# lastdancewithyou/multimodal_edema_prediction

Measured on AMD Instinct MI355X. Metric: multimodal train samples/sec, higher is better.
Workload: dtype bf16

## Files before the change

multimodal_edema_prediction_amd/csrc/elementwise.hip:

```cpp
#include "common.h"
#include "medp_hip.h"

namespace {

__global__ __launch_bounds__(256) void cast_f32_bf16_kernel(const float* __restrict__ x, int ldx, bf16_t* __restrict__ y, int ldy,
                                                            int rows, int cols) {
    const int c4 = cols >> 2;
    const size_t total = (size_t)rows * c4;
    for (size_t i = (size_t)blockIdx.x * 256 + threadIdx.x; i < total; i += (size_t)gridDim.x * 256) {
        const int r = (int)(i / c4), c = (int)(i % c4) * 4;
        const float4 v = *(const float4*)(x + (size_t)r * ldx + c);
        uint2 o;
        o.x = pack_bf2(v.x, v.y);
        o.y = pack_bf2(v.z, v.w);
        *(uint2*)(y + (size_t)r * ldy + c) = o;
    }
}

template <typename TIN>
__global__ __launch_bounds__(256) void transpose_to_bf16_kernel(const TIN* __restrict__ x, int ldx, bf16_t* __restrict__ y, int ldy,
                                                                int rows, int cols) {
    __shared__ float tile[64][65];
    const int r0 = blockIdx.y * 64, c0 = blockIdx.x * 64;
    const int tx = threadIdx.x & 63, ty = threadIdx.x >> 6;
    for (int i = ty; i < 64; i += 4) {
        const int r = r0 + i, c = c0 + tx;
        float v = 0.f;
        if (r < rows && c < cols) {
            if constexpr (sizeof(TIN) == 2) v = bf2f(((const bf16_t*)x)[(size_t)r * ldx + c]);
            else v = ((const float*)x)[(size_t)r * ldx + c];
        }
        tile[i][tx] = v;
    }
    __syncthreads();
    for (int i = ty; i < 64; i += 4) {
        const int c = c0 + i, r = r0 + tx;
        if (c < cols && r < rows) y[(size_t)c * ldy + r] = f2bf(tile[tx][i]);
    }
}

__global__ __launch_bounds__(256) void weight_operands_multi_kernel(const MedpOperandJob* __restrict__ jobs, const int* __restrict__ blk_job,
                                                                    const int* __restrict__ blk_tile) {
    __shared__ float tile[64][65];
    const MedpOperandJob j = jobs[blk_job[blockIdx.x]];
    const int tiles_c = (j.cols + 63) / 64;
    const int t = blk_tile[blockIdx.x];
    const int r0 = (t / tiles_c) * 64, c0 = (t % tiles_c) * 64;
    const int tx = threadIdx.x & 63, ty = threadIdx.x >> 6;
    const float* x = (const float*)j.src;
    bf16_t* yp = (bf16_t*)j.dst_plain;
    bf16_t* yt = (bf16_t*)j.dst_t;
    for (int i = ty; i < 64; i += 4) {
        const int r = r0 + i, c = c0 + tx;
        float v = 0.f;
        if (r < j.rows && c < j.cols) {
            v = x[(size_t)r * j.ld_src + c];
            if (yp) yp[(size_t)r * j.ld_plain + c] = f2bf(v);
        }
        tile[i][tx] = v;
    }
    if (!yt) return;
    __syncthreads();
    for (int i = ty; i < 64; i += 4) {
        const int c = c0 + i, r = r0 + tx;
        if (c < j.cols && r < j.rows) yt[(size_t)c * j.ld_t + r] = f2bf(tile[tx][i]);
    }
}

__global__ __launch_bounds__(256) void gelu_bwd_kernel(const float* __restrict__ dy, const float* __restrict__ pre, float* __restrict__ dx,
                                                       size_t n) {
    for (size_t i = ((size_t)blockIdx.x * 256 + threadIdx.x) * 4; i < n; i += (size_t)gridDim.x * 1024) {
        const float4 g = *(const float4*)(dy + i), p = *(const float4*)(pre + i);
        *(float4*)(dx + i) = make_float4(g.x * gelu_erf_grad(p.x), g.y * gelu_erf_grad(p.y), g.z * gelu_erf_grad(p.z),
                                         g.w * gelu_erf_grad(p.w));
    }
}

__global__ __launch_bounds__(256) void gelu_bf16_fwd_kernel(const bf16_t* __restrict__ pre, bf16_t* __restrict__ out, size_t n8) {
    for (size_t i = (size_t)blockIdx.x * 256 + threadIdx.x; i < n8; i += (size_t)gridDim.x * 256) {
        const uint4 p = *(const uint4*)(pre + i * 8);
        const uint32_t w[4] = {p.x, p.y, p.z, p.w};
        uint32_t o[4];
#pragma unroll
        for (int k = 0; k < 4; ++k) {
            const f32x2 g = gelu_erf2((f32x2){__uint_as_float(w[k] << 16), __uint_as_float(w[k] & 0xffff0000u)});
            o[k] = pack_bf2(g[0], g[1]);
        }
        *(uint4*)(out + i * 8) = make_uint4(o[0], o[1], o[2], o[3]);
    }
}
__global__ __launch_bounds__(256) void gelu_bf16_bwd_kernel(const bf16_t* __restrict__ dy, const bf16_t* __restrict__ pre,
                                                            bf16_t* __restrict__ dx, size_t n8) {
    for (size_t i = (size_t)blockIdx.x * 256 + threadIdx.x; i < n8; i += (size_t)gridDim.x * 256) {
        const uint4 g = *(const uint4*)(dy + i * 8), p = *(const uint4*)(pre + i * 8);
        const uint32_t gw[4] = {g.x, g.y, g.z, g.w}, pw[4] = {p.x, p.y, p.z, p.w};
        uint32_t o[4];
#pragma unroll
        for (int k = 0; k < 4; ++k) {
            const float a = __uint_as_float(gw[k] << 16) * gelu_erf_grad(__uint_as_float(pw[k] << 16));
            const float b = __uint_as_float(gw[k] & 0xffff0000u) * gelu_erf_grad(__uint_as_float(pw[k] & 0xffff0000u));
            o[k] = pack_bf2(a, b);
        }
        *(uint4*)(dx + i * 8) = make_uint4(o[0], o[1], o[2], o[3]);
    }
}

__global__ __launch_bounds__(256) void im2col_patch_kernel(const float* __restrict__ pix, bf16_t* __restrict__ A, int B, int C, int H,
                                                           int W, int ps, int kpad) {
    const unsigned gh = H / ps, gw = W / ps, K = C * ps * ps, pp = ps * ps, k8 = kpad >> 3;
    const unsigned total = (unsigned)B * gh * gw * k8;
    for (unsigned i = blockIdx.x * 256u + threadIdx.x; i < total; i += gridDim.x * 256u) {
        const unsigned kc = i % k8, row = i / k8;
        const unsigned px = row % gw, r2 = row / gw, py = r2 % gh, b = r2 / gh;
        const float* img = pix + (size_t)b * C * H * W + (size_t)(py * ps) * W + px * ps;
        float v[8];
#pragma unroll
        for (int u = 0; u < 8; ++u) {
            const unsigned kk = kc * 8 + u;
            float x = 0.f;
            if (kk < K) {
                const unsigned c = kk / pp, rem = kk - c * pp, ii = rem / ps, jj = rem - ii * ps;
                x = img[((size_t)c * H + ii) * W + jj];
            }
            v[u] = x;
        }
        uint4 o;
        o.x = pack_bf2(v[0], v[1]);
        o.y = pack_bf2(v[2], v[3]);
        o.z = pack_bf2(v[4], v[5]);
        o.w = pack_bf2(v[6], v[7]);
        *(uint4*)(A + (size_t)row * kpad + kc * 8) = o;
    }
}

__global__ __launch_bounds__(256) void vit_assemble_kernel(const float* __restrict__ patch, const float* __restrict__ cls,
                                                           const float* __restrict__ pos, float* __restrict__ x, int B, int P, int D) {
    const int d4 = D >> 2;
    const size_t total = (size_t)B * (P + 1) * d4;
    for (size_t i = (size_t)blockIdx.x * 256 + threadIdx.x; i < total; i += (size_t)gridDim.x * 256) {
        const int c = (int)(i % d4) * 4;
        const size_t tokrow = i / d4;
        const int t = (int)(tokrow % (P + 1)), b = (int)(tokrow / (P + 1));
        const float4 pe = *(const float4*)(pos + (size_t)t * D + c);
        const float4 v = (t == 0) ? *(const float4*)(cls + c) : *(const float4*)(patch + ((size_t)b * P + t - 1) * D + c);
        *(float4*)(x + tokrow * D + c) = make_float4(v.x + pe.x, v.y + pe.y, v.z + pe.z, v.w + pe.w);
    }
}

__device__ __forceinline__ float cubic1(float x, float A) { return ((A + 2.f) * x - (A + 3.f)) * x * x + 1.f; }
__device__ __forceinline__ float cubic2(float x, float A) { return ((A * x - 5.f * A) * x + 8.f * A) * x - 4.f * A; }
__global__ __launch_bounds__(256) void pos_bicubic_kernel(const float* __restrict__ pos, float* __restrict__ out, int s, int gh, int gw,
                                                          int D) {
    const size_t total = (size_t)(gh * gw + 1) * D;
    const float A = -0.75f;
    for (size_t i = (size_t)blockIdx.x * 256 + threadIdx.x; i < total; i += (size_t)gridDim.x * 256) {
        const int d = (int)(i % D), t = (int)(i / D);
        if (t == 0) { out[i] = pos[d]; continue; }
        const int oy = (t - 1) / gw, ox = (t - 1) % gw;
        const float sy = (float)s / (float)gh, sx = (float)s / (float)gw;
        const float fy = (oy + 0.5f) * sy - 0.5f, fx = (ox + 0.5f) * sx - 0.5f;
        const int iy = (int)floorf(fy), ix = (int)floorf(fx);
        const float ty = fy - iy, tx = fx - ix;
        const float wy[4] = {cubic2(ty + 1.f, A), cubic1(ty, A), cubic1(1.f - ty, A), cubic2(2.f - ty, A)};
        const float wx[4] = {cubic2(tx + 1.f, A), cubic1(tx, A), cubic1(1.f - tx, A), cubic2(2.f - tx, A)};
        float acc = 0.f;
#pragma unroll
        for (int a = 0; a < 4; ++a) {
            const int yy = min(max(iy - 1 + a, 0), s - 1);
            float rowacc = 0.f;
#pragma unroll
            for (int c = 0; c < 4; ++c) {
                const int xx = min(max(ix - 1 + c, 0), s - 1);
                rowacc += wx[c] * pos[(size_t)(1 + yy * s + xx) * D + d];
            }
            acc += wy[a] * rowacc;
        }
        out[i] = acc;
    }
}

__device__ __forceinline__ float bicubic_tap_weight(int src, int dst, int s, int g) {
    const float A = -0.75f;
    const float sc = (float)s / (float)g;
    const float f = (dst + 0.5f) * sc - 0.5f;
    const int i0 = (int)floorf(f);
    const float t = f - i0;
    const float w[4] = {cubic2(t + 1.f, A), cubic1(t, A), cubic1(1.f - t, A), cubic2(2.f - t, A)};
    float acc = 0.f;
#pragma unroll
    for (int a = 0; a < 4; ++a)
        if (min(max(i0 - 1 + a, 0), s - 1) == src) acc += w[a];
    return acc;
}
__global__ __launch_bounds__(256) void pos_bicubic_bwd_kernel(const float* __restrict__ dout, float* __restrict__ dpos, int s, int gh,
                                                              int gw, int D) {
    const int d4n = D >> 2;
    const int total = (s * s + 1) * d4n;
    for (int i = blockIdx.x * 256 + threadIdx.x; i < total; i += gridDim.x * 256) {
        const int d4 = i % d4n, cell = i / d4n;
        if (cell == 0) {
            *(float4*)(dpos + 4 * d4) = *(const float4*)(dout + 4 * d4);
            continue;
        }
        const int sy = (cell - 1) / s, sx = (cell - 1) % s;
        float4 acc = make_float4(0.f, 0.f, 0.f, 0.f);
        for (int oy = 0; oy < gh; ++oy) {
            const float wy = bicubic_tap_weight(sy, oy, s, gh);
            if (wy == 0.f) continue;
            for (int ox = 0; ox < gw; ++ox) {
                const float wx = bicubic_tap_weight(sx, ox, s, gw);
                if (wx == 0.f) continue;
                const float w = wy * wx;
                const float4 g = *(const float4*)(dout + (size_t)(1 + oy * gw + ox) * D + 4 * d4);
                acc.x += w * g.x; acc.y += w * g.y; acc.z += w * g.z; acc.w += w * g.w;
            }
        }
        *(float4*)(dpos + (size_t)cell * D + 4 * d4) = acc;
    }
}

inline int grid_for(size_t work_items) { return (int)min((size_t)4096, max((size_t)1, (work_items + 255) / 256)); }

}

extern "C" int medp_cast_f32_bf16(const float* x, int ldx, void* y, int ldy, int rows, int cols, void* stream) {
    MEDP_CHECK_ARG(x && y && rows > 0 && cols > 0, "cast: bad argument");
    MEDP_CHECK_ARG(cols % 4 == 0 && ldx % 4 == 0 && ldy % 4 == 0, "cast: cols, ldx, ldy must be multiples of 4");
    cast_f32_bf16_kernel<<<grid_for((size_t)rows * cols / 4), 256, 0, (hipStream_t)stream>>>(x, ldx, (bf16_t*)y, ldy, rows, cols);
    MEDP_LAUNCH_CHECK("medp_cast_f32_bf16");
    return 0;
}

extern "C" int medp_transpose_to_bf16(const void* x, int x_is_bf16, int ldx, void* y, int ldy, int rows, int cols, void* stream) {
    MEDP_CHECK_ARG(x && y && rows > 0 && cols > 0 && ldx >= cols && ldy >= rows, "transpose: bad argument");
    dim3 grid((cols + 63) / 64, (rows + 63) / 64);
    if (x_is_bf16)
        transpose_to_bf16_kernel<bf16_t><<<grid, 256, 0, (hipStream_t)stream>>>((const bf16_t*)x, ldx, (bf16_t*)y, ldy, rows, cols);
    else
        transpose_to_bf16_kernel<float><<<grid, 256, 0, (hipStream_t)stream>>>((const float*)x, ldx, (bf16_t*)y, ldy, rows, cols);
    MEDP_LAUNCH_CHECK("medp_transpose_to_bf16");
    return 0;
}

extern "C" int medp_weight_operands_multi(const MedpOperandJob* dev_jobs, const int* dev_block_job, const int* dev_block_tile, int n_blocks,
                                          void* stream) {
    MEDP_CHECK_ARG(dev_jobs && dev_block_job && dev_block_tile && n_blocks > 0, "weight_operands_multi: bad argument");
    weight_operands_multi_kernel<<<n_blocks, 256, 0, (hipStream_t)stream>>>(dev_jobs, dev_block_job, dev_block_tile);
    MEDP_LAUNCH_CHECK("medp_weight_operands_multi");
    return 0;
}

extern "C" int medp_gelu_bwd(const float* dy, const float* pre, float* dx, long long n, void* stream) {
    MEDP_CHECK_ARG(dy && pre && dx && n > 0 && n % 4 == 0, "gelu_bwd: bad argument (n must be a multiple of 4)");
    gelu_bwd_kernel<<<grid_for((size_t)n / 4), 256, 0, (hipStream_t)stream>>>(dy, pre, dx, (size_t)n);
    MEDP_LAUNCH_CHECK("medp_gelu_bwd");
    return 0;
}

extern "C" int medp_gelu_bf16_fwd(const void* pre, void* out, long long n, void* stream) {
    MEDP_CHECK_ARG(pre && out && n > 0 && n % 8 == 0, "gelu_bf16_fwd: bad argument (n must be a multiple of 8)");
    gelu_bf16_fwd_kernel<<<grid_for((size_t)n / 8), 256, 0, (hipStream_t)stream>>>((const bf16_t*)pre, (bf16_t*)out, (size_t)n / 8);
    MEDP_LAUNCH_CHECK("medp_gelu_bf16_fwd");
    return 0;
}

extern "C" int medp_gelu_bf16_bwd(const void* dy, const void* pre, void* dx, long long n, void* stream) {
    MEDP_CHECK_ARG(dy && pre && dx && n > 0 && n % 8 == 0, "gelu_bf16_bwd: bad argument (n must be a multiple of 8)");
    gelu_bf16_bwd_kernel<<<grid_for((size_t)n / 8), 256, 0, (hipStream_t)stream>>>((const bf16_t*)dy, (const bf16_t*)pre, (bf16_t*)dx,
                                                                                  (size_t)n / 8);
    MEDP_LAUNCH_CHECK("medp_gelu_bf16_bwd");
    return 0;
}

extern "C" int medp_im2col_patch(const float* pix, void* A, int B, int C, int H, int W, int patch, int kpad, void* stream) {
    MEDP_CHECK_ARG(pix && A && B > 0 && C > 0 && patch > 0, "im2col: bad argument");
    MEDP_CHECK_ARG(H >= patch && W >= patch, "im2col: image %dx%d smaller than the patch size %d", H, W, patch);
    MEDP_CHECK_ARG(kpad >= C * patch * patch && kpad % 8 == 0, "im2col: kpad must be >= C*p*p and a multiple of 8");
    const size_t total = (size_t)B * (H / patch) * (W / patch) * (kpad / 8);
    MEDP_CHECK_ARG(total < (1ull << 31), "im2col: B * patches * kpad / 8 must stay below 2^31");
    im2col_patch_kernel<<<grid_for(total), 256, 0, (hipStream_t)stream>>>(pix, (bf16_t*)A, B, C, H, W, patch, kpad);
    MEDP_LAUNCH_CHECK("medp_im2col_patch");
    return 0;
}

extern "C" int medp_vit_assemble(const float* patch, const float* cls, const float* pos, float* x, int B, int P, int D, void* stream) {
    MEDP_CHECK_ARG(patch && cls && pos && x && B > 0 && P > 0 && D % 4 == 0, "vit_assemble: bad argument");
    vit_assemble_kernel<<<grid_for((size_t)B * (P + 1) * D / 4), 256, 0, (hipStream_t)stream>>>(patch, cls, pos, x, B, P, D);
    MEDP_LAUNCH_CHECK("medp_vit_assemble");
    return 0;
}

extern "C" int medp_pos_embed_bicubic_bwd(const float* dout, float* dpos, int src_side, int gh, int gw, int D, void* stream) {
    MEDP_CHECK_ARG(dout && dpos && src_side > 0 && gh > 0 && gw > 0 && D > 0 && D % 4 == 0, "pos_embed_bicubic_bwd: bad argument");
    pos_bicubic_bwd_kernel<<<grid_for((size_t)(src_side * src_side + 1) * (D / 4)), 256, 0, (hipStream_t)stream>>>(dout, dpos, src_side, gh, gw, D);
    MEDP_LAUNCH_CHECK("medp_pos_embed_bicubic_bwd");
    return 0;
}

extern "C" int medp_pos_embed_bicubic(const float* pos, float* out, int src_side, int gh, int gw, int D, void* stream) {
    MEDP_CHECK_ARG(pos && out && src_side > 0 && gh > 0 && gw > 0 && D > 0, "pos_embed_bicubic: bad argument");
    pos_bicubic_kernel<<<grid_for((size_t)(gh * gw + 1) * D), 256, 0, (hipStream_t)stream>>>(pos, out, src_side, gh, gw, D);
    MEDP_LAUNCH_CHECK("medp_pos_embed_bicubic");
    return 0;
}
```

multimodal_edema_prediction_amd/csrc/norm.hip:

```cpp
#include <stdlib.h>

#include "common.h"
#include "medp_hip.h"

namespace {

template <bool OUT_BF16>
__global__ __launch_bounds__(256) void layernorm_fwd_kernel(const float* __restrict__ x, int ldx, const float* __restrict__ w,
                                                            const float* __restrict__ b, void* __restrict__ y, int ldy,
                                                            float* __restrict__ mean_out, float* __restrict__ rstd_out,
                                                            int rows, int D, float eps) {
    const int lane = threadIdx.x & 63;
    const int row = blockIdx.x * 4 + (threadIdx.x >> 6);
    if (row >= rows) return;
    const float* xr = x + (size_t)row * ldx;
    const int D4 = D >> 2;
    float s = 0.f;
    for (int i = lane; i < D4; i += 64) {
        const float4 v = *(const float4*)(xr + 4 * i);
        s += (v.x + v.y) + (v.z + v.w);
    }
    const float mean = wave_sum(s) / (float)D;
    float ss = 0.f;
    for (int i = lane; i < D4; i += 64) {
        const float4 v = *(const float4*)(xr + 4 * i);
        const float a = v.x - mean, c = v.y - mean, d = v.z - mean, e = v.w - mean;
        ss += (a * a + c * c) + (d * d + e * e);
    }
    const float rstd = rsqrtf(wave_sum(ss) / (float)D + eps);
    if (lane == 0) {
        if (mean_out) mean_out[row] = mean;
        if (rstd_out) rstd_out[row] = rstd;
    }
    for (int i = lane; i < D4; i += 64) {
        const float4 v = *(const float4*)(xr + 4 * i);
        const float4 ww = *(const float4*)(w + 4 * i);
        const float4 bb = *(const float4*)(b + 4 * i);
        const float o0 = (v.x - mean) * rstd * ww.x + bb.x, o1 = (v.y - mean) * rstd * ww.y + bb.y;
        const float o2 = (v.z - mean) * rstd * ww.z + bb.z, o3 = (v.w - mean) * rstd * ww.w + bb.w;
        if (OUT_BF16) {
            uint2 o;
            o.x = pack_bf2(o0, o1);
            o.y = pack_bf2(o2, o3);
            *(uint2*)((bf16_t*)y + (size_t)row * ldy + 4 * i) = o;
        } else {
            *(float4*)((float*)y + (size_t)row * ldy + 4 * i) = make_float4(o0, o1, o2, o3);
        }
    }
}

template <bool OUT_BF16, int NV>
__global__ __launch_bounds__(256) void layernorm_fwd_reg_kernel(const float* __restrict__ x, int ldx, const float* __restrict__ w,
                                                                const float* __restrict__ b, void* __restrict__ y, int ldy,
                                                                float* __restrict__ mean_out, float* __restrict__ rstd_out,
                                                                int rows, float eps) {
    constexpr int D = 256 * NV;
    const int lane = threadIdx.x & 63;
    const int row = blockIdx.x * 4 + (threadIdx.x >> 6);
    if (row >= rows) return;
    const float* xr = x + (size_t)row * ldx;
    float4 v[NV];
#pragma unroll
    for (int j = 0; j < NV; ++j) v[j] = *(const float4*)(xr + 4 * (lane + 64 * j));
    float s = 0.f;
#pragma unroll
    for (int j = 0; j < NV; ++j) s += (v[j].x + v[j].y) + (v[j].z + v[j].w);
    const float mean = wave_sum(s) / (float)D;
    float ss = 0.f;
#pragma unroll
    for (int j = 0; j < NV; ++j) {
        const float a = v[j].x - mean, c = v[j].y - mean, d = v[j].z - mean, e = v[j].w - mean;
        ss += (a * a + c * c) + (d * d + e * e);
    }
    const float rstd = rsqrtf(wave_sum(ss) / (float)D + eps);
    if (lane == 0) {
        if (mean_out) mean_out[row] = mean;
        if (rstd_out) rstd_out[row] = rstd;
    }
#pragma unroll
    for (int j = 0; j < NV; ++j) {
        const int i = lane + 64 * j;
        const float4 ww = *(const float4*)(w + 4 * i);
        const float4 bb = *(const float4*)(b + 4 * i);
        const float o0 = (v[j].x - mean) * rstd * ww.x + bb.x, o1 = (v[j].y - mean) * rstd * ww.y + bb.y;
        const float o2 = (v[j].z - mean) * rstd * ww.z + bb.z, o3 = (v[j].w - mean) * rstd * ww.w + bb.w;
        if (OUT_BF16) {
            uint2 o;
            o.x = pack_bf2(o0, o1);
            o.y = pack_bf2(o2, o3);
            *(uint2*)((bf16_t*)y + (size_t)row * ldy + 4 * i) = o;
        } else {
            *(float4*)((float*)y + (size_t)row * ldy + 4 * i) = make_float4(o0, o1, o2, o3);
        }
    }
}

__global__ __launch_bounds__(256) void layernorm_bwd_dx_kernel(const float* __restrict__ dy, int lddy, const float* __restrict__ x,
                                                               int ldx, const float* __restrict__ w, const float* __restrict__ mean,
                                                               const float* __restrict__ rstd, float* __restrict__ dx, int lddx,
                                                               int rows, int D, int accumulate) {
    const int lane = threadIdx.x & 63;
    const int row = blockIdx.x * 4 + (threadIdx.x >> 6);
    if (row >= rows) return;
    const float* xr = x + (size_t)row * ldx;
    const float* gr = dy + (size_t)row * lddy;
    const float mu = mean[row], rs = rstd[row];
    const int D4 = D >> 2;
    float s1 = 0.f, s2 = 0.f;
    for (int i = lane; i < D4; i += 64) {
        const float4 v = *(const float4*)(xr + 4 * i), g = *(const float4*)(gr + 4 * i), ww = *(const float4*)(w + 4 * i);
        const float g0 = g.x * ww.x, g1 = g.y * ww.y, g2 = g.z * ww.z, g3 = g.w * ww.w;
        s1 += (g0 + g1) + (g2 + g3);
        s2 += (g0 * (v.x - mu) + g1 * (v.y - mu)) + (g2 * (v.z - mu) + g3 * (v.w - mu));
    }
    s1 = wave_sum(s1) / (float)D;
    s2 = wave_sum(s2) * rs / (float)D;
    float* dr = dx + (size_t)row * lddx;
    for (int i = lane; i < D4; i += 64) {
        const float4 v = *(const float4*)(xr + 4 * i), g = *(const float4*)(gr + 4 * i), ww = *(const float4*)(w + 4 * i);
        float4 o;
        o.x = rs * (g.x * ww.x - s1 - (v.x - mu) * rs * s2);
        o.y = rs * (g.y * ww.y - s1 - (v.y - mu) * rs * s2);
        o.z = rs * (g.z * ww.z - s1 - (v.z - mu) * rs * s2);
        o.w = rs * (g.w * ww.w - s1 - (v.w - mu) * rs * s2);
        if (accumulate) {
            const float4 old = *(const float4*)(dr + 4 * i);
            o.x += old.x; o.y += old.y; o.z += old.z; o.w += old.w;
        }
        *(float4*)(dr + 4 * i) = o;
    }
}

template <int MODE>
__global__ __launch_bounds__(256) void colsum_partial_kernel(const float* __restrict__ dy, int lddy, const float* __restrict__ x, int ldx,
                                                             const float* __restrict__ mean, const float* __restrict__ rstd,
                                                             float* __restrict__ partial, int rows, int D, int rows_per_chunk) {
    __shared__ float red[2][4][64];
    const int cl = threadIdx.x & 63, rl = threadIdx.x >> 6;
    const int c = blockIdx.x * 64 + cl;
    const int chunk = blockIdx.y, nchunk = gridDim.y;
    const int r0 = chunk * rows_per_chunk, r1 = min(rows, r0 + rows_per_chunk);
    float a = 0.f, bsum = 0.f;
    if (c < D) {
        for (int r = r0 + rl; r < r1; r += 4) {
            const float g = dy[(size_t)r * lddy + c];
            bsum += g;
            if (MODE == 1) a += g * (x[(size_t)r * ldx + c] - mean[r]) * rstd[r];
        }
    }
    red[0][rl][cl] = a;
    red[1][rl][cl] = bsum;
    __syncthreads();
    if (rl == 0 && c < D) {
        if (MODE == 1) partial[(size_t)chunk * D + c] = (red[0][0][cl] + red[0][1][cl]) + (red[0][2][cl] + red[0][3][cl]);
        partial[(size_t)(nchunk + chunk) * D + c] = (red[1][0][cl] + red[1][1][cl]) + (red[1][2][cl] + red[1][3][cl]);
    }
}

__global__ __launch_bounds__(256) void colsum_final_kernel(const float* __restrict__ partial, float* __restrict__ out_a,
                                                           float* __restrict__ out_b, int nchunk, int D) {
    __shared__ float red[2][4][64];
    const int cl = threadIdx.x & 63, kl = threadIdx.x >> 6;
    const int c = blockIdx.x * 64 + cl;
    float a = 0.f, b = 0.f;
    if (c < D) {
#pragma unroll 4
        for (int k = kl; k < nchunk; k += 4) {
            if (out_a) a += partial[(size_t)k * D + c];
            b += partial[(size_t)(nchunk + k) * D + c];
        }
    }
    red[0][kl][cl] = a;
    red[1][kl][cl] = b;
    __syncthreads();
    if (kl == 0 && c < D) {
        if (out_a) out_a[c] = (red[0][0][cl] + red[0][1][cl]) + (red[0][2][cl] + red[0][3][cl]);
        if (out_b) out_b[c] = (red[1][0][cl] + red[1][1][cl]) + (red[1][2][cl] + red[1][3][cl]);
    }
}

template <bool OUT_BF16>
__global__ __launch_bounds__(256) void scalenorm_fwd_kernel(const float* __restrict__ x, int ldx, const float* __restrict__ g,
                                                            void* __restrict__ y, int ldy, float* __restrict__ rnorm_out, int rows,
                                                            int D, float eps) {
    const int lane = threadIdx.x & 63;
    const int row = blockIdx.x * 4 + (threadIdx.x >> 6);
    if (row >= rows) return;
    const float* xr = x + (size_t)row * ldx;
    const int D4 = D >> 2;
    float ss = 0.f;
    for (int i = lane; i < D4; i += 64) {
        const float4 v = *(const float4*)(xr + 4 * i);
        ss += (v.x * v.x + v.y * v.y) + (v.z * v.z + v.w * v.w);
    }
    const float rn = 1.0f / fmaxf(sqrtf(wave_sum(ss)), eps);
    if (lane == 0 && rnorm_out) rnorm_out[row] = rn;
    const float sc = rn * sqrtf((float)D) * g[0];
    for (int i = lane; i < D4; i += 64) {
        const float4 v = *(const float4*)(xr + 4 * i);
        if (OUT_BF16) {
            uint2 o;
            o.x = pack_bf2(v.x * sc, v.y * sc);
            o.y = pack_bf2(v.z * sc, v.w * sc);
            *(uint2*)((bf16_t*)y + (size_t)row * ldy + 4 * i) = o;
        } else {
            *(float4*)((float*)y + (size_t)row * ldy + 4 * i) = make_float4(v.x * sc, v.y * sc, v.z * sc, v.w * sc);
        }
    }
}

template <bool OUT_BF16, int NV>
__global__ __launch_bounds__(256) void scalenorm_fwd_reg_kernel(const float* __restrict__ x, int ldx, const float* __restrict__ g,
                                                                void* __restrict__ y, int ldy, float* __restrict__ rnorm_out,
                                                                int rows, int D, float eps) {
    const int lane = threadIdx.x & 63;
    const int row = blockIdx.x * 4 + (threadIdx.x >> 6);
    if (row >= rows) return;
    const float* xr = x + (size_t)row * ldx;
    const int D4 = D >> 2;
    float4 v[NV];
#pragma unroll
    for (int k = 0; k < NV; ++k) {
        const int i = lane + 64 * k;
        v[k] = i < D4 ? *(const float4*)(xr + 4 * i) : make_float4(0.f, 0.f, 0.f, 0.f);
    }
    float ss = 0.f;
#pragma unroll
    for (int k = 0; k < NV; ++k)
        if (lane + 64 * k < D4) ss += (v[k].x * v[k].x + v[k].y * v[k].y) + (v[k].z * v[k].z + v[k].w * v[k].w);
    const float rn = 1.0f / fmaxf(sqrtf(wave_sum(ss)), eps);
    if (lane == 0 && rnorm_out) rnorm_out[row] = rn;
    const float sc = rn * sqrtf((float)D) * g[0];
#pragma unroll
    for (int k = 0; k < NV; ++k) {
        const int i = lane + 64 * k;
        if (i < D4) {
            if (OUT_BF16) {
                uint2 o;
                o.x = pack_bf2(v[k].x * sc, v[k].y * sc);
                o.y = pack_bf2(v[k].z * sc, v[k].w * sc);
                *(uint2*)((bf16_t*)y + (size_t)row * ldy + 4 * i) = o;
            } else {
                *(float4*)((float*)y + (size_t)row * ldy + 4 * i) = make_float4(v[k].x * sc, v[k].y * sc, v[k].z * sc, v[k].w * sc);
            }
        }
    }
}

__global__ __launch_bounds__(256) void scalenorm_bwd_kernel(const float* __restrict__ dy, int lddy, const float* __restrict__ x, int ldx,
                                                            const float* __restrict__ g, const float* __restrict__ rnorm, const float* acc_src,
                                                            int ldacc, float* dx, int lddx, float* dg_rows, int rows, int D) {
    const int lane = threadIdx.x & 63;
    const int row = blockIdx.x * 4 + (threadIdx.x >> 6);
    if (row >= rows) return;
    {
        const float* xr = x + (size_t)row * ldx;
        const float* gr = dy + (size_t)row * lddy;
        const int D4 = D >> 2;
        float dot = 0.f;
        for (int i = lane; i < D4; i += 64) {
            const float4 v = *(const float4*)(xr + 4 * i), d = *(const float4*)(gr + 4 * i);
            dot += (v.x * d.x + v.y * d.y) + (v.z * d.z + v.w * d.w);
        }
        dot = wave_sum(dot);
        const float rn = rnorm[row], sq = sqrtf((float)D);
        if (lane == 0 && dg_rows) dg_rows[row] = sq * rn * dot;
        const float s = sq * g[0] * rn, k = rn * rn * dot;
        float* dr = dx + (size_t)row * lddx;
        for (int i = lane; i < D4; i += 64) {
            const float4 v = *(const float4*)(xr + 4 * i), d = *(const float4*)(gr + 4 * i);
            float4 o = make_float4(s * (d.x - v.x * k), s * (d.y - v.y * k), s * (d.z - v.z * k), s * (d.w - v.w * k));
            if (acc_src) {
                const float4 old = *(const float4*)(acc_src + (size_t)row * ldacc + 4 * i);
                o.x += old.x; o.y += old.y; o.z += old.z; o.w += old.w;
            }
            *(float4*)(dr + 4 * i) = o;
        }
    }
}

template <int NV>
__global__ __launch_bounds__(256) void scalenorm_bwd_reg_kernel(const float* __restrict__ dy, int lddy, const float* __restrict__ x, int ldx,
                                                                const float* __restrict__ g, const float* __restrict__ rnorm,
                                                                const float* acc_src, int ldacc, float* dx, int lddx, float* dg_rows, int rows,
                                                                int D) {
    const int lane = threadIdx.x & 63;
    const int row = blockIdx.x * 4 + (threadIdx.x >> 6);
    if (row >= rows) return;
    {
        const float* xr = x + (size_t)row * ldx;
        const float* gr = dy + (size_t)row * lddy;
        const int D4 = D >> 2;
        float4 v[NV], d[NV];
        float dot = 0.f;
#pragma unroll
        for (int j = 0; j < NV; ++j) {
            const int i = lane + 64 * j;
            const bool ok = i < D4;
            v[j] = ok ? *(const float4*)(xr + 4 * i) : make_float4(0.f, 0.f, 0.f, 0.f);
            d[j] = ok ? *(const float4*)(gr + 4 * i) : make_float4(0.f, 0.f, 0.f, 0.f);
        }
#pragma unroll
        for (int j = 0; j < NV; ++j) dot += (v[j].x * d[j].x + v[j].y * d[j].y) + (v[j].z * d[j].z + v[j].w * d[j].w);
        dot = wave_sum(dot);
        const float rn = rnorm[row], sq = sqrtf((float)D);
        if (lane == 0 && dg_rows) dg_rows[row] = sq * rn * dot;
        const float s = sq * g[0] * rn, k = rn * rn * dot;
        float* dr = dx + (size_t)row * lddx;
#pragma unroll
        for (int j = 0; j < NV; ++j) {
            const int i = lane + 64 * j;
            if (i < D4) {
                float4 o = make_float4(s * (d[j].x - v[j].x * k), s * (d[j].y - v[j].y * k), s * (d[j].z - v[j].z * k), s * (d[j].w - v[j].w * k));
                if (acc_src) {
                    const float4 old = *(const float4*)(acc_src + (size_t)row * ldacc + 4 * i);
                    o.x += old.x; o.y += old.y; o.z += old.z; o.w += old.w;
                }
                *(float4*)(dr + 4 * i) = o;
            }
        }
    }
}

__global__ __launch_bounds__(256) void sum_all_kernel(const float* __restrict__ v, float* __restrict__ out, int n) {
    __shared__ float red[4];
    float s = 0.f;
    for (int i = threadIdx.x; i < n; i += 256) s += v[i];
    s = wave_sum(s);
    if ((threadIdx.x & 63) == 0) red[threadIdx.x >> 6] = s;
    __syncthreads();
    if (threadIdx.x == 0) out[0] = (red[0] + red[1]) + (red[2] + red[3]);
}

int colsum_chunks(int rows) { return max(1, min(128, rows / 64)); }

constexpr int COLSUM_DIRECT_MAX_ROWS = 2048;
template <int MODE>
__global__ __launch_bounds__(1024) void colsum_direct_kernel(const float* __restrict__ dy, int lddy, const float* __restrict__ x, int ldx,
                                                            const float* __restrict__ mean, const float* __restrict__ rstd,
                                                            float* __restrict__ out_a, float* __restrict__ out_b, int rows, int D) {
    __shared__ float red[2][16][64];
    const int cl = threadIdx.x & 63, rl = threadIdx.x >> 6;
    const int c = blockIdx.x * 64 + cl;
    float a = 0.f, bsum = 0.f;
    if (c < D) {
#pragma unroll 4
        for (int r = rl; r < rows; r += 16) {
            const float g = dy[(size_t)r * lddy + c];
            bsum += g;
            if (MODE == 1) a += g * (x[(size_t)r * ldx + c] - mean[r]) * rstd[r];
        }
    }
    red[0][rl][cl] = a;
    red[1][rl][cl] = bsum;
    __syncthreads();
    if (rl == 0 && c < D) {
        float sa = 0.f, sb = 0.f;
#pragma unroll
        for (int k = 0; k < 16; ++k) {
            sa += red[0][k][cl];
            sb += red[1][k][cl];
        }
        if (MODE == 1 && out_a) out_a[c] = sa;
        if (out_b) out_b[c] = sb;
    }
}

}

extern "C" int medp_layernorm_fwd(const float* x, int ldx, const float* w, const float* b, void* y, int ldy, int y_bf16,
                                  float* mean, float* rstd, int rows, int D, float eps, void* stream) {
    MEDP_CHECK_ARG(x && w && b && y, "layernorm_fwd: null operand");
    MEDP_CHECK_ARG(rows > 0 && D > 0 && D % 4 == 0 && ldx % 4 == 0 && ldy % 4 == 0, "layernorm_fwd: D, ldx, ldy must be multiples of 4");
    dim3 grid((rows + 3) / 4);
    hipStream_t s = (hipStream_t)stream;
    if (D == 768 && y_bf16)
        layernorm_fwd_reg_kernel<true, 3><<<grid, 256, 0, s>>>(x, ldx, w, b, y, ldy, mean, rstd, rows, eps);
    else if (D == 768)
        layernorm_fwd_reg_kernel<false, 3><<<grid, 256, 0, s>>>(x, ldx, w, b, y, ldy, mean, rstd, rows, eps);
    else if (D == 256 && y_bf16)
        layernorm_fwd_reg_kernel<true, 1><<<grid, 256, 0, s>>>(x, ldx, w, b, y, ldy, mean, rstd, rows, eps);
    else if (D == 256)
        layernorm_fwd_reg_kernel<false, 1><<<grid, 256, 0, s>>>(x, ldx, w, b, y, ldy, mean, rstd, rows, eps);
    else if (y_bf16)
        layernorm_fwd_kernel<true><<<grid, 256, 0, s>>>(x, ldx, w, b, y, ldy, mean, rstd, rows, D, eps);
    else
        layernorm_fwd_kernel<false><<<grid, 256, 0, s>>>(x, ldx, w, b, y, ldy, mean, rstd, rows, D, eps);
    MEDP_LAUNCH_CHECK("medp_layernorm_fwd");
    return 0;
}

extern "C" size_t medp_colsum_workspace_bytes(int rows, int D) { return (size_t)2 * colsum_chunks(rows) * D * sizeof(float); }

extern "C" int medp_layernorm_bwd(const float* dy, int lddy, const float* x, int ldx, const float* w, const float* mean,
                                  const float* rstd, float* dx, int lddx, int accumulate_dx, float* dw, float* db,
                                  float* workspace, int rows, int D, void* stream) {
    MEDP_CHECK_ARG(dy && x && w && mean && rstd, "layernorm_bwd: null operand");
    MEDP_CHECK_ARG(rows > 0 && D > 0 && D % 4 == 0 && ldx % 4 == 0 && lddy % 4 == 0 && lddx % 4 == 0, "layernorm_bwd: alignment");
    hipStream_t s = (hipStream_t)stream;
    if (dx) {
        layernorm_bwd_dx_kernel<<<(rows + 3) / 4, 256, 0, s>>>(dy, lddy, x, ldx, w, mean, rstd, dx, lddx, rows, D, accumulate_dx);
        MEDP_LAUNCH_CHECK("medp_layernorm_bwd(dx)");
    }
    if (dw || db) {
        MEDP_CHECK_ARG(workspace, "layernorm_bwd: workspace required for dw/db (medp_colsum_workspace_bytes)");
        if (rows <= COLSUM_DIRECT_MAX_ROWS) {
            colsum_direct_kernel<1><<<(D + 63) / 64, 1024, 0, s>>>(dy, lddy, x, ldx, mean, rstd, dw, db, rows, D);
            MEDP_LAUNCH_CHECK("medp_layernorm_bwd(direct)");
            return 0;
        }
        const int nchunk = colsum_chunks(rows), rpc = (rows + nchunk - 1) / nchunk;
        colsum_partial_kernel<1><<<dim3((D + 63) / 64, nchunk), 256, 0, s>>>(dy, lddy, x, ldx, mean, rstd, workspace, rows, D, rpc);
        MEDP_LAUNCH_CHECK("medp_layernorm_bwd(partial)");
        colsum_final_kernel<<<(D + 63) / 64, 256, 0, s>>>(workspace, dw, db, nchunk, D);
        MEDP_LAUNCH_CHECK("medp_layernorm_bwd(final)");
    }
    return 0;
}

extern "C" int medp_colsum_f32(const float* x, int ldx, float* out, float* workspace, int rows, int D, void* stream) {
    MEDP_CHECK_ARG(x && out && workspace && rows > 0 && D > 0, "colsum: bad argument");
    hipStream_t s = (hipStream_t)stream;
    if (rows <= COLSUM_DIRECT_MAX_ROWS) {
        colsum_direct_kernel<0><<<(D + 63) / 64, 1024, 0, s>>>(x, ldx, nullptr, 0, nullptr, nullptr, nullptr, out, rows, D);
        MEDP_LAUNCH_CHECK("medp_colsum_f32(direct)");
        return 0;
    }
    const int nchunk = colsum_chunks(rows), rpc = (rows + nchunk - 1) / nchunk;
    colsum_partial_kernel<0><<<dim3((D + 63) / 64, nchunk), 256, 0, s>>>(x, ldx, nullptr, 0, nullptr, nullptr, workspace, rows, D, rpc);
    MEDP_LAUNCH_CHECK("medp_colsum_f32(partial)");
    colsum_final_kernel<<<(D + 63) / 64, 256, 0, s>>>(workspace, nullptr, out, nchunk, D);
    MEDP_LAUNCH_CHECK("medp_colsum_f32(final)");
    return 0;
}

extern "C" int medp_scalenorm_fwd(const float* x, int ldx, const float* g, void* y, int ldy, int y_bf16, float* rnorm, int rows,
                                  int D, float eps, void* stream) {
    MEDP_CHECK_ARG(x && g && y, "scalenorm_fwd: null operand");
    MEDP_CHECK_ARG(rows > 0 && D > 0 && D % 4 == 0 && ldx % 4 == 0 && ldy % 4 == 0, "scalenorm_fwd: D, ldx, ldy must be multiples of 4");
    dim3 grid((rows + 3) / 4);
    const int nv = (D / 4 + 63) / 64;
    hipStream_t st = (hipStream_t)stream;
#define MEDP_SN_REG(NV)                                                                                             \
    do {                                                                                                            \
        if (y_bf16) scalenorm_fwd_reg_kernel<true, NV><<<grid, 256, 0, st>>>(x, ldx, g, y, ldy, rnorm, rows, D, eps);  \
        else scalenorm_fwd_reg_kernel<false, NV><<<grid, 256, 0, st>>>(x, ldx, g, y, ldy, rnorm, rows, D, eps);       \
    } while (0)
    if (nv <= 2) MEDP_SN_REG(2);
    else if (nv <= 5) MEDP_SN_REG(5);
    else if (nv <= 10) MEDP_SN_REG(10);
    else if (nv <= 16) MEDP_SN_REG(16);
    else if (y_bf16)
        scalenorm_fwd_kernel<true><<<grid, 256, 0, st>>>(x, ldx, g, y, ldy, rnorm, rows, D, eps);
    else
        scalenorm_fwd_kernel<false><<<grid, 256, 0, st>>>(x, ldx, g, y, ldy, rnorm, rows, D, eps);
#undef MEDP_SN_REG
    MEDP_LAUNCH_CHECK("medp_scalenorm_fwd");
    return 0;
}

static int scalenorm_bwd_launch(const float* dy, int lddy, const float* x, int ldx, const float* g, const float* rnorm, const float* acc_src,
                                int ldacc, float* dx, int lddx, float* dg, float* workspace_rows, int rows, int D, void* stream) {
    MEDP_CHECK_ARG(dy && x && g && rnorm && dx, "scalenorm_bwd: null operand");
    MEDP_CHECK_ARG(rows > 0 && D % 4 == 0 && ldx % 4 == 0 && lddy % 4 == 0 && lddx % 4 == 0 && ldacc % 4 == 0, "scalenorm_bwd: alignment");
    MEDP_CHECK_ARG(!dg || workspace_rows, "scalenorm_bwd: dg needs a rows-float workspace");
    hipStream_t s = (hipStream_t)stream;
    const int nv = (D / 4 + 63) / 64;
    float* dgr = dg ? workspace_rows : nullptr;
    const int grid = (rows + 3) / 4;
    if (nv <= 5) scalenorm_bwd_reg_kernel<5><<<grid, 256, 0, s>>>(dy, lddy, x, ldx, g, rnorm, acc_src, ldacc, dx, lddx, dgr, rows, D);
    else if (nv <= 10) scalenorm_bwd_reg_kernel<10><<<grid, 256, 0, s>>>(dy, lddy, x, ldx, g, rnorm, acc_src, ldacc, dx, lddx, dgr, rows, D);
    else scalenorm_bwd_kernel<<<grid, 256, 0, s>>>(dy, lddy, x, ldx, g, rnorm, acc_src, ldacc, dx, lddx, dgr, rows, D);
    MEDP_LAUNCH_CHECK("medp_scalenorm_bwd");
    if (dg) {
        sum_all_kernel<<<1, 256, 0, s>>>(workspace_rows, dg, rows);
        MEDP_LAUNCH_CHECK("medp_scalenorm_bwd(dg)");
    }
    return 0;
}

extern "C" int medp_scalenorm_bwd(const float* dy, int lddy, const float* x, int ldx, const float* g, const float* rnorm, float* dx,
                                  int lddx, int accumulate_dx, float* dg, float* workspace_rows, int rows, int D, void* stream) {
    return scalenorm_bwd_launch(dy, lddy, x, ldx, g, rnorm, accumulate_dx ? dx : nullptr, lddx, dx, lddx, dg, workspace_rows, rows, D, stream);
}

extern "C" int medp_scalenorm_bwd_add(const float* dy, int lddy, const float* x, int ldx, const float* g, const float* rnorm, const float* add,
                                      int ldadd, float* dx, int lddx, float* dg, float* workspace_rows, int rows, int D, void* stream) {
    MEDP_CHECK_ARG(add, "scalenorm_bwd_add: null operand");
    return scalenorm_bwd_launch(dy, lddy, x, ldx, g, rnorm, add, ldadd, dx, lddx, dg, workspace_rows, rows, D, stream);
}
```

Measured before the change: 12580.

## Add specialized patch-14 im2col and optional pipelined multi-row LayerNorm forward

Adds an im2col kernel specialized for patch size 14 that reads float2 pairs with incremental index stepping instead of per-element div/mod, enabled by default through an env variable. Also adds a persistent, software-pipelined LayerNorm forward kernel that processes multiple rows per wave, stages weights in shared memory, and can pair bf16 stores across lanes with DPP. That kernel is gated behind an env variable that defaults off. Both paths add debug hooks for choosing the variant at runtime.

```diff
diff --git a/multimodal_edema_prediction_amd/csrc/elementwise.hip b/multimodal_edema_prediction_amd/csrc/elementwise.hip
--- a/multimodal_edema_prediction_amd/csrc/elementwise.hip
+++ b/multimodal_edema_prediction_amd/csrc/elementwise.hip
@@ -133,6 +133,33 @@
     }
 }
 
+__global__ __launch_bounds__(256) void im2col_patch14_kernel(const float* __restrict__ pix, bf16_t* __restrict__ A, int B, int C, int H,
+                                                             int W, int kpad) {
+    constexpr unsigned PS = 14, PP = PS * PS;
+    const unsigned gh = H / PS, gw = W / PS, K = C * PP, k8 = kpad >> 3;
+    const unsigned total = (unsigned)B * gh * gw * k8;
+    for (unsigned i = blockIdx.x * 256u + threadIdx.x; i < total; i += gridDim.x * 256u) {
+        const unsigned kc = i % k8, row = i / k8;
+        const unsigned px = row % gw, r2 = row / gw, py = r2 % gh, b = r2 / gh;
+        const float* img = pix + (size_t)b * C * H * W + (size_t)(py * PS) * W + px * PS;
+        const unsigned k0 = kc * 8;
+        unsigned c = k0 / PP, ii = (k0 - c * PP) / PS, jj = k0 - c * PP - ii * PS;
+        uint32_t o[4];
+#pragma unroll
+        for (int u = 0; u < 4; ++u) {
+            float2 v = make_float2(0.f, 0.f);
+            if (k0 + 2 * u < K) v = *(const float2*)(img + ((size_t)c * H + ii) * W + jj);
+            o[u] = pack_bf2(v.x, v.y);
+            jj += 2;
+            if (jj == PS) {
+                jj = 0;
+                if (++ii == PS) { ii = 0; ++c; }
+            }
+        }
+        *(uint4*)(A + (size_t)row * kpad + k0) = make_uint4(o[0], o[1], o[2], o[3]);
+    }
+}
+
 __global__ __launch_bounds__(256) void vit_assemble_kernel(const float* __restrict__ patch, const float* __restrict__ cls,
                                                            const float* __restrict__ pos, float* __restrict__ x, int B, int P, int D) {
     const int d4 = D >> 2;
@@ -272,13 +299,28 @@
     return 0;
 }
 
+static int g_im2col_variant = -1;
+static int im2col_env_variant() {
+    static const int v = [] { const char* e = getenv("MEDP_IM2COL_PAIRS"); return e ? atoi(e) : 1; }();
+    return v;
+}
+extern "C" int medp_dbg_im2col_variant(int v) {
+    const int prev = g_im2col_variant;
+    g_im2col_variant = v;
+    return prev;
+}
+
 extern "C" int medp_im2col_patch(const float* pix, void* A, int B, int C, int H, int W, int patch, int kpad, void* stream) {
     MEDP_CHECK_ARG(pix && A && B > 0 && C > 0 && patch > 0, "im2col: bad argument");
     MEDP_CHECK_ARG(H >= patch && W >= patch, "im2col: image %dx%d smaller than the patch size %d", H, W, patch);
     MEDP_CHECK_ARG(kpad >= C * patch * patch && kpad % 8 == 0, "im2col: kpad must be >= C*p*p and a multiple of 8");
     const size_t total = (size_t)B * (H / patch) * (W / patch) * (kpad / 8);
     MEDP_CHECK_ARG(total < (1ull << 31), "im2col: B * patches * kpad / 8 must stay below 2^31");
-    im2col_patch_kernel<<<grid_for(total), 256, 0, (hipStream_t)stream>>>(pix, (bf16_t*)A, B, C, H, W, patch, kpad);
+    const int variant = g_im2col_variant >= 0 ? g_im2col_variant : im2col_env_variant();
+    if (variant > 0 && patch == 14 && W % 2 == 0 && ((uintptr_t)pix & 7) == 0)
+        im2col_patch14_kernel<<<grid_for(total), 256, 0, (hipStream_t)stream>>>(pix, (bf16_t*)A, B, C, H, W, kpad);
+    else
+        im2col_patch_kernel<<<grid_for(total), 256, 0, (hipStream_t)stream>>>(pix, (bf16_t*)A, B, C, H, W, patch, kpad);
     MEDP_LAUNCH_CHECK("medp_im2col_patch");
     return 0;
 }
diff --git a/multimodal_edema_prediction_amd/csrc/norm.hip b/multimodal_edema_prediction_amd/csrc/norm.hip
--- a/multimodal_edema_prediction_amd/csrc/norm.hip
+++ b/multimodal_edema_prediction_amd/csrc/norm.hip
@@ -91,6 +91,141 @@
             *(uint2*)((bf16_t*)y + (size_t)row * ldy + 4 * i) = o;
         } else {
             *(float4*)((float*)y + (size_t)row * ldy + 4 * i) = make_float4(o0, o1, o2, o3);
+        }
+    }
+}
+
+template <int NV, int R>
+__device__ __forceinline__ void ln_pipe_load(float4 (&v)[R][NV], const float* __restrict__ x, int ldx, int row0, int lane) {
+#pragma unroll
+    for (int r = 0; r < R; ++r) {
+        const float* xr = x + (size_t)(row0 + r) * ldx;
+#pragma unroll
+        for (int j = 0; j < NV; ++j) v[r][j] = *(const float4*)(xr + 4 * (lane + 64 * j));
+    }
+}
+
+template <bool OUT_BF16, int NV, int R, bool PAIR16>
+__device__ __forceinline__ void ln_pipe_rows(const float4 (&v)[R][NV], const float4* sw, const float4* sb, void* __restrict__ y, int ldy,
+                                             float* __restrict__ mean_out, float* __restrict__ rstd_out, int row0, float eps, int lane) {
+#pragma clang fp contract(off)
+    constexpr int D = 256 * NV;
+    float mean[R], rstd[R];
+#pragma unroll
+    for (int r = 0; r < R; ++r) {
+        float s = 0.f;
+#pragma unroll
+        for (int j = 0; j < NV; ++j) s += (v[r][j].x + v[r][j].y) + (v[r][j].z + v[r][j].w);
+        mean[r] = wave_sum(s) / (float)D;
+        float ss = 0.f;
+#pragma unroll
+        for (int j = 0; j < NV; ++j) {
+            const float a = v[r][j].x - mean[r], c = v[r][j].y - mean[r], d = v[r][j].z - mean[r], e = v[r][j].w - mean[r];
+            if (NV == 1 || j < 2) ss += __builtin_fmaf(a, a, c * c) + __builtin_fmaf(d, d, e * e);
+            else ss += (a * a + c * c) + (d * d + e * e);
+        }
+        rstd[r] = rsqrtf(wave_sum(ss) / (float)D + eps);
+        if (lane == 0) {
+            if (mean_out) mean_out[row0 + r] = mean[r];
+            if (rstd_out) rstd_out[row0 + r] = rstd[r];
+        }
+    }
+    int li = lane;
+    asm volatile("" : "+v"(li));
+#pragma unroll
+    for (int j = 0; j < NV; ++j) {
+        const int i = lane + 64 * j;
+        const float4 ww = sw[li + 64 * j];
+        const float4 bb = sb[li + 64 * j];
+        uint2 pk[R];
+#pragma unroll
+        for (int r = 0; r < R; ++r) {
+            const float o0 = __builtin_fmaf((v[r][j].x - mean[r]) * rstd[r], ww.x, bb.x);
+            const float o1 = __builtin_fmaf((v[r][j].y - mean[r]) * rstd[r], ww.y, bb.y);
+            const float o2 = __builtin_fmaf((v[r][j].z - mean[r]) * rstd[r], ww.z, bb.z);
+            const float o3 = __builtin_fmaf((v[r][j].w - mean[r]) * rstd[r], ww.w, bb.w);
+            if constexpr (!OUT_BF16) {
+                *(float4*)((float*)y + (size_t)(row0 + r) * ldy + 4 * i) = make_float4(o0, o1, o2, o3);
+            } else {
+                pk[r].x = pack_bf2(o0, o1);
+                pk[r].y = pack_bf2(o2, o3);
+                if constexpr (!PAIR16) *(uint2*)((bf16_t*)y + (size_t)(row0 + r) * ldy + 4 * i) = pk[r];
+            }
+        }
+        if constexpr (PAIR16) {
+            const int odd = lane & 1;
+#pragma unroll
+            for (int r = 0; r < R; r += 2) {
+                const uint2 give = odd ? pk[r] : pk[r + 1];
+                uint2 got;
+                got.x = (uint32_t)__builtin_amdgcn_mov_dpp((int)give.x, 0xB1, 0xF, 0xF, true);
+                got.y = (uint32_t)__builtin_amdgcn_mov_dpp((int)give.y, 0xB1, 0xF, 0xF, true);
+                const uint4 o = odd ? make_uint4(got.x, got.y, pk[r + 1].x, pk[r + 1].y) : make_uint4(pk[r].x, pk[r].y, got.x, got.y);
+                *(uint4*)((bf16_t*)y + (size_t)(row0 + r + odd) * ldy + 4 * (i - odd)) = o;
+            }
+        }
+    }
+}
+
+constexpr int ln_pipe_min_waves(int NV, int R, bool PREFETCH) {
+    const int row_regs = 4 * NV * R * (PREFETCH ? 2 : 1);
+    return row_regs <= 12 ? 8 : row_regs <= 24 ? 6 : 4;
+}
+template <bool OUT_BF16, int NV, int R, bool PREFETCH, bool PAIR16>
+__global__ __launch_bounds__(256, ln_pipe_min_waves(NV, R, PREFETCH)) void layernorm_fwd_pipe_kernel(
+    const float* __restrict__ x, int ldx, const float* __restrict__ w, const float* __restrict__ b, void* __restrict__ y, int ldy,
+    float* __restrict__ mean_out, float* __restrict__ rstd_out, int rows, float eps) {
+    static_assert(!PAIR16 || (OUT_BF16 && R % 2 == 0), "paired stores need bf16 output and an even number of rows");
+    const int lane = threadIdx.x & 63;
+    const int W = gridDim.x * 4, wave = blockIdx.x * 4 + (threadIdx.x >> 6), groups = rows / R;
+    __shared__ float4 sw[64 * NV], sb[64 * NV];
+    float4 fw, fb;
+    if (threadIdx.x < 64 * NV) {
+        fw = *(const float4*)(w + 4 * threadIdx.x);
+        fb = *(const float4*)(b + 4 * threadIdx.x);
+    }
+    float4 va[R][NV], vb[R][NV];
+    int g = wave;
+    if (g < groups) ln_pipe_load<NV, R>(va, x, ldx, g * R, lane);
+    if (threadIdx.x < 64 * NV) {
+        sw[threadIdx.x] = fw;
+        sb[threadIdx.x] = fb;
+    }
+    __syncthreads();
+    if (g < groups) {
+        for (;;) {
+            const int g1 = g + W;
+            if constexpr (!PREFETCH) {
+                ln_pipe_rows<OUT_BF16, NV, R, PAIR16>(va, sw, sb, y, ldy, mean_out, rstd_out, g * R, eps, lane);
+                if (g1 >= groups) break;
+                ln_pipe_load<NV, R>(va, x, ldx, g1 * R, lane);
+                g = g1;
+            } else {
+                if (g1 >= groups) {
+                    ln_pipe_rows<OUT_BF16, NV, R, PAIR16>(va, sw, sb, y, ldy, mean_out, rstd_out, g * R, eps, lane);
+                    break;
+                }
+                ln_pipe_load<NV, R>(vb, x, ldx, g1 * R, lane);
+                __builtin_amdgcn_sched_barrier(0);
+                ln_pipe_rows<OUT_BF16, NV, R, PAIR16>(va, sw, sb, y, ldy, mean_out, rstd_out, g * R, eps, lane);
+                g = g1 + W;
+                if (g >= groups) {
+                    ln_pipe_rows<OUT_BF16, NV, R, PAIR16>(vb, sw, sb, y, ldy, mean_out, rstd_out, g1 * R, eps, lane);
+                    break;
+                }
+                ln_pipe_load<NV, R>(va, x, ldx, g * R, lane);
+                __builtin_amdgcn_sched_barrier(0);
+                ln_pipe_rows<OUT_BF16, NV, R, PAIR16>(vb, sw, sb, y, ldy, mean_out, rstd_out, g1 * R, eps, lane);
+            }
+        }
+    }
+    if constexpr (R > 1) {
+        if (wave == groups % W) {
+            for (int row = groups * R; row < rows; ++row) {
+                float4 vt[1][NV];
+                ln_pipe_load<NV, 1>(vt, x, ldx, row, lane);
+                ln_pipe_rows<OUT_BF16, NV, 1, false>(vt, sw, sb, y, ldy, mean_out, rstd_out, row, eps, lane);
+            }
         }
     }
 }
@@ -366,7 +501,58 @@
     }
 }
 
-}
+constexpr int LN_PIPE_MIN_ROWS = 8192;
+int g_ln_variant = -1;
+int g_ln_grid_cap = 0;
+int ln_env_variant() {
+    static const int v = [] { const char* e = getenv("MEDP_LN_PIPELINED"); return e ? atoi(e) : 0; }();
+    return v;
+}
+int ln_cu_count() {
+    static const int cus = [] { int dev = 0, n = 256; (void)hipGetDevice(&dev); (void)hipDeviceGetAttribute(&n, hipDeviceAttributeMultiprocessorCount, dev); return n; }();
+    return cus;
+}
+
+template <bool OUT_BF16, int NV, int R, bool PREFETCH, bool PAIR16>
+void ln_pipe_launch(const float* x, int ldx, const float* w, const float* b, void* y, int ldy, float* mean, float* rstd, int rows, float eps,
+                    hipStream_t s) {
+    const int need = (rows / R + (rows % R ? 1 : 0) + 3) / 4;
+    int grid = need;
+    if (PREFETCH) {
+        const int cap = ln_cu_count() * ln_pipe_min_waves(NV, R, PREFETCH), sweeps = (need + cap - 1) / cap;
+        grid = (need + sweeps - 1) / sweeps;
+    }
+    if (g_ln_grid_cap > 0) grid = min(grid, g_ln_grid_cap);
+    layernorm_fwd_pipe_kernel<OUT_BF16, NV, R, PREFETCH, PAIR16><<<grid, 256, 0, s>>>(x, ldx, w, b, y, ldy, mean, rstd, rows, eps);
+}
+
+template <int NV>
+void ln_pipe_dispatch(int variant, const float* x, int ldx, const float* w, const float* b, void* y, int ldy, int y_bf16, float* mean,
+                      float* rstd, int rows, float eps, hipStream_t s) {
+    if (variant == 1) {
+        const bool pair_ok = ldy % 8 == 0 && ((uintptr_t)y & 15) == 0;
+        if (y_bf16 && pair_ok) ln_pipe_launch<true, NV, 2, false, true>(x, ldx, w, b, y, ldy, mean, rstd, rows, eps, s);
+        else if (y_bf16) ln_pipe_launch<true, NV, 2, false, false>(x, ldx, w, b, y, ldy, mean, rstd, rows, eps, s);
+        else ln_pipe_launch<false, NV, 2, false, false>(x, ldx, w, b, y, ldy, mean, rstd, rows, eps, s);
+    } else {
+        if (y_bf16) ln_pipe_launch<true, NV, 1, true, false>(x, ldx, w, b, y, ldy, mean, rstd, rows, eps, s);
+        else ln_pipe_launch<false, NV, 1, true, false>(x, ldx, w, b, y, ldy, mean, rstd, rows, eps, s);
+    }
+}
+
+}
+
+extern "C" int medp_dbg_layernorm_variant(int v) {
+    const int prev = g_ln_variant;
+    g_ln_variant = v;
+    return prev;
+}
+extern "C" int medp_dbg_layernorm_grid(int n) {
+    const int prev = g_ln_grid_cap;
+    g_ln_grid_cap = n;
+    return prev;
+}
+extern "C" int medp_dbg_layernorm_rows_per_workgroup(int v) { return v == 1 ? 8 : 4; }
 
 extern "C" int medp_layernorm_fwd(const float* x, int ldx, const float* w, const float* b, void* y, int ldy, int y_bf16,
                                   float* mean, float* rstd, int rows, int D, float eps, void* stream) {
@@ -374,6 +560,13 @@
     MEDP_CHECK_ARG(rows > 0 && D > 0 && D % 4 == 0 && ldx % 4 == 0 && ldy % 4 == 0, "layernorm_fwd: D, ldx, ldy must be multiples of 4");
     dim3 grid((rows + 3) / 4);
     hipStream_t s = (hipStream_t)stream;
+    const int variant = g_ln_variant >= 0 ? g_ln_variant : (rows >= LN_PIPE_MIN_ROWS ? ln_env_variant() : 0);
+    if (variant > 0 && (D == 768 || D == 256)) {
+        if (D == 768) ln_pipe_dispatch<3>(variant, x, ldx, w, b, y, ldy, y_bf16, mean, rstd, rows, eps, s);
+        else ln_pipe_dispatch<1>(variant, x, ldx, w, b, y, ldy, y_bf16, mean, rstd, rows, eps, s);
+        MEDP_LAUNCH_CHECK("medp_layernorm_fwd(pipelined)");
+        return 0;
+    }
     if (D == 768 && y_bf16)
         layernorm_fwd_reg_kernel<true, 3><<<grid, 256, 0, s>>>(x, ldx, w, b, y, ldy, mean, rstd, rows, eps);
     else if (D == 768)
```

Result: no change. 12580 (-0.0%).
